# DavidBluecame/libYafaRay

Hardware: AMD Instinct MI355X
Metric: Mrays/sec + Msamples/sec, 1920×1080×64spp path-trace at 1/2/4/8 GPUs (higher is better)
Workload: dtype f32

## Files before the change

libyafaray_amd/csrc/devscene.h:

```cpp
#pragma once
#include <cstdint>
#include <hip/hip_runtime.h>

namespace yafamd
{
struct DevStats;

struct RadGrid
{
	const uint32_t *start;
	const float4 *pos;
	const float4 *dir;
	float lo[3];
	float cell, inv_cell;
	int nx, ny, nz;
};

enum : uint32_t
{
	B_NONE = 0, B_SPECULAR = 1u << 0, B_GLOSSY = 1u << 1, B_DIFFUSE = 1u << 2, B_DISPERSIVE = 1u << 3,
	B_REFLECT = 1u << 4, B_TRANSMIT = 1u << 5, B_FILTER = 1u << 6, B_EMIT = 1u << 7, B_VOLUMETRIC = 1u << 8,
	B_ALL = B_SPECULAR | B_GLOSSY | B_DIFFUSE | B_DISPERSIVE | B_REFLECT | B_TRANSMIT | B_FILTER
};

// ... 287 lines not shown
	float4 *pcol;
	float4 *pwo;
	float4 *pend_thr;
	float4 *pend_emit;
	float4 *v0p;
	float4 *v0wo;
	uint4 *pr;
	float4 *csmp;
	float *nee;
	float *nee_aw;
	uint8_t *occ;
	float4 *ts;
	float4 *v0attr;
};

struct DevQueues
{
	int *slot;
	float *ray_o;
	float *ray_d;
	float2 *ray_tt;
	float tmin_dflt;
	float *hit_t;
	int *hit_prim;
	float4 *sh_o;
	float4 *sh_d;
	int *sh_idx;
	float2 *ts_hit;
	int *ts_n;
	float4 *sattr;
	const uint32_t *perm;
	int trace_part;
	int nee_grid;
};

enum : int
{
	TRACE_BOTH = 0,
	TRACE_CLOSEST = 1,
	TRACE_SHADOW = 2,
};

struct DevNeeQueue
{
	float4 *p_prim;
	float4 *wo_k;
	uint4 *pix_mode;
	float4 *attr;
	float4 *extra;
};

enum : uint32_t
{
	G_DIFFUSE = 1u,
	G_CAUSTIC = 2u,
	G_EXTRA = 4u,
	G_FG = 8u,
	G_SHOWMAP = 16u,
};

struct PhotonState
{
	float4 *ray_o;
	float4 *ray_d;
	float4 *pcol;
	uint32_t *alive[2];
// ... 81 lines not shown
```

libyafaray_amd/csrc/kernels.hip:

```cpp

#include <atomic>
#include <hip/hip_runtime.h>
#include <cstdlib>
#include <string>
#include "devmath.h"
#include "photonheap.h"
#include "devscene.h"
#include "texeval.h"

namespace yafamd
{

#ifndef YAF_TRACE_BLOCK
#define YAF_TRACE_BLOCK 128
#endif
#ifndef YAF_SHADE_MIN_WAVES
#define YAF_SHADE_MIN_WAVES 4
#endif
#ifndef YAF_SHADE_LEAN_WAVES
#define YAF_SHADE_LEAN_WAVES 4
#endif
#ifndef YAF_SHADE_PREFETCH
#define YAF_SHADE_PREFETCH 1
#endif
// ... 761 lines not shown
			if(pk[1] != 0xffffffffu) { push((int)(pk[1] & nm)); ++sp; }
			next = pk[0] != 0xffffffffu ? (int)(pk[0] & nm) : -1;
		}
		else if constexpr(!YAF_CLOSEST_SORT)
		{
			int kmin = 0;
#pragma unroll
			for(int k = 1; k < 4; ++k) kmin = key[k] < key[kmin] ? k : kmin;
			next = key[kmin] < inf ? child[kmin] : -1;
#pragma unroll
			for(int k = 3; k >= 0; --k)
				if(k != kmin && key[k] < inf) { push(child[k]); ++sp; }
		}
		else
		{
			cswap(key[0], child[0], key[1], child[1]);
			cswap(key[2], child[2], key[3], child[3]);
			cswap(key[0], child[0], key[2], child[2]);
			cswap(key[1], child[1], key[3], child[3]);
			cswap(key[1], child[1], key[2], child[2]);
			if(key[3] < inf) { push(child[3]); ++sp; }
			if(key[2] < inf) { push(child[2]); ++sp; }
			if(key[1] < inf) { push(child[1]); ++sp; }
			next = key[0] < inf ? child[0] : -1;
		}
		if(next < 0)
		{
			if(sp == 0) break;
			--sp;
			next = (!SPILL || sp < C.lds_depth) ? C.stack[sp * kTraceBlock + YAF_LANE]
			                                    : C.spill[(uint32_t)(sp - C.lds_depth) * C.spill_stride + glane];
		}
		node = next;
	}
	return prim_best >= 0;
}

#undef YAF_LANE

template<bool SPILL, bool STATS = true>
__device__ void traceRefill4(const TraceCtx &C, const DevQueues &Q, const DevPaths &P, uint32_t n_a, uint32_t total,
                             uint32_t a0, uint32_t s0, uint32_t j, uint32_t stride, uint32_t &visits, uint32_t &tests,
                             uint32_t &n_closest, uint32_t &n_shadow)
{
	const int lane = threadIdx.x;
	const uint32_t glane = blockIdx.x * blockDim.x + threadIdx.x;
	const float inf = __builtin_huge_valf();
	V3 o = v3(0.f, 0.f, 0.f), d = o, id = o, oid = o;
	SlabSel sel{0, 2, 4};
	float tmin = 0.f, tmax = 0.f, box_t0 = 0.f, t_best = 0.f;
	int prim_best = -1, sp = 0, node = -1;
	bool any = false;
	uint32_t cur = 0;
	auto push = [&](int v) {
		if(sp < C.lds_depth) C.stack[sp * kTraceBlock + lane] = v;
		else if(SPILL) C.spill[(uint32_t)(sp - C.lds_depth) * C.spill_stride + glane] = v;
	};
	for(;;)
	{
		if(node < 0)
		{
			bool got = false;
			for(;;)
			{
				if(j >= total) break;
				cur = j;
// ... 396 lines not shown
	{
		const uint32_t k = key[r];
		uint64_t m = ~0ull;
#pragma unroll
		for(int b = 0; b < 6; ++b)
		{
			const bool bit = (k >> b) & 1u;
			const uint64_t bal = __ballot(bit);
			m &= bit ? bal : ~bal;
		}
		const uint32_t below = (uint32_t)__popcll(m & lt);
		const uint32_t old = W.base[k];
		off[r] = old + below;
		__builtin_amdgcn_wave_barrier();
		if(below == 0) W.base[k] = old + (uint32_t)__popcll(m);
		__builtin_amdgcn_wave_barrier();
	}
	const uint32_t c = W.base[lane];
	uint32_t inc = c;
#pragma unroll
	for(int o = 1; o < 64; o <<= 1)
	{
		const uint32_t v = __shfl_up(inc, o);
		if(lane >= o) inc += v;
	}
	__builtin_amdgcn_wave_barrier();
	W.base[lane] = inc - c;
	__builtin_amdgcn_wave_barrier();
#pragma unroll
	for(int r = 0; r < kSortPer; ++r) W.perm[W.base[key[r]] + off[r]] = (uint16_t)(r * 64 + lane);
	__builtin_amdgcn_wave_barrier();
}

template<bool LDS_SCENE, bool WIDE, bool TS, bool SPILL = true, bool STATS = true, bool SORT = false, bool W8 = false>
__global__ void __launch_bounds__(kTraceBlock) YAF_TRACE_ATTR k_trace(DevScene S, DevQueues Q, DevCounters cnt, DevPaths P,
                                                      DevStats *stats, int stack_depth, int *spill)
{
	extern __shared__ float4 smem[];
	int *stack = reinterpret_cast<int *>(smem);
	TraceCtx C;
	C.wave_base = waveBase();
	C.stack = stack;
	C.lds_depth = stack_depth;
	C.spill = spill;
	C.spill_stride = gridDim.x * blockDim.x;
	if(LDS_SCENE)
	{
		float4 *lds_nodes = smem + (stack_depth * kTraceBlock) / 4;
		float4 *lds_tris = lds_nodes + S.node_f4 * S.n_nodes;
		for(int k = threadIdx.x; k < S.node_f4 * S.n_nodes; k += blockDim.x) lds_nodes[k] = S.nodes[k];
		for(int k = threadIdx.x; k < 3 * S.n_tris; k += blockDim.x) lds_tris[k] = S.tris[k];
		__syncthreads();
		C.nodes = lds_nodes;
		C.tris = lds_tris;
	}
	else
	{
		C.nodes = S.nodes;
		C.tris = S.tris;
		if constexpr(W8)
		{
			C.nodes = S.nodes8;
			C.tris = S.tris8;
			if(S.lds_top8 > 0)
			{
				float4 *top = smem + (stack_depth * kTraceBlock) / 4;
				for(int k = threadIdx.x; k < 5 * S.lds_top8; k += blockDim.x) top[(k / 5) * kTop8Stride + (k % 5)] = S.nodes8[8 * (k / 5) + (k % 5)];
				__syncthreads();
				C.top = top;
				C.n_top = S.lds_top8;
			}
		}
		else if(WIDE && S.lds_top > 0)
		{
			float4 *top = smem + (stack_depth * kTraceBlock) / 4;
			for(int k = threadIdx.x; k < 8 * S.lds_top; k += blockDim.x) top[(k >> 3) * kTopStride + (k & 7)] = S.nodes[k];
			__syncthreads();
			C.top = top;
			C.n_top = S.lds_top;
		}
	}
	const SegLoop L = segLoop(S.n_seg);
	const uint32_t n_a = cnt.n_active[L.s], n_s = Q.trace_part == TRACE_CLOSEST ? 0u : cnt.n_shadow[L.s];
	const uint32_t total = n_a + n_s;
	const uint32_t j_first = Q.trace_part == TRACE_SHADOW ? n_a : 0u;
	const uint32_t a0 = L.s * S.cap_a, s0 = L.s * S.cap_s;
	uint32_t visits = 0, tests = 0, n_closest = 0, n_shadow = 0;
	uint32_t w_closest = 0, w_shadow = 0;
	auto countWave = [&](int kind) {
		w_closest += (uint32_t)__popcll(__ballot(kind == 1));
		w_shadow += (uint32_t)__popcll(__ballot(kind == 2));
	};
	const uint32_t stride = L.nb * blockDim.x;
	auto traceEntry = [&](uint32_t j) -> int {
		if(j < n_a)
		{
			const uint32_t i = a0 + j;
			V3 o, d;
			float tmin, tw;
			if(loadQRay(Q, i, o, d, tmin, tw))
			{
				float t;
				int prim;
				const float tmax = (tw >= 0.f) ? tw : __builtin_huge_valf();
				traverse<false, WIDE, SPILL, false, STATS, LDS_SCENE>(C, o, d, tmin, tmax, t, prim, visits, tests);
				raySt(&Q.hit_t[i], t);
				raySt(&Q.hit_prim[i], prim);
				return 1;
			}
		}
		else if(j < total)
		{
			const uint32_t k = s0 + (j - n_a);
			const float4 od = rayLd4(&Q.sh_o[k]), dd = rayLd4(&Q.sh_d[k]);
			float t;
			int prim;
			bool occ;
			if(TS)
			{
				TsList L;
				L.hit = Q.ts_hit + (size_t)k * (uint32_t)S.s_depth;
				L.n = 0;
				L.cap = S.s_depth;
				L.prim_ng = S.prim_ng;
				L.mats = S.mats;
				occ = traverse<true, WIDE, SPILL, true>(C, xyz(od), xyz(dd), od.w, dd.w, t, prim, visits, tests, &L);
				Q.ts_n[k] = occ ? 0 : L.n;
			}
			else occ = traverse<true, WIDE, SPILL, false, STATS>(C, xyz(od), xyz(dd), 0.f, dd.w, t, prim, visits, tests);
			P.occ[TS ? Q.sh_idx[k] : __float_as_int(od.w)] = occ ? 1 : 0;
			return 2;
		}
		return 0;
	};
	if constexpr(SORT)
	{
		__shared__ WaveSort wsort[kTraceBlock / 64];
		WaveSort &W = wsort[threadIdx.x >> 6];
		const uint32_t nwv = blockDim.x >> 6;
		const uint32_t gw = L.r * nwv + (threadIdx.x >> 6), nw = L.nb * nwv;
		for(uint32_t w0 = gw * kSortWin; w0 < total; w0 += nw * kSortWin)
		{
			uint32_t key[kSortPer];
#pragma unroll
			for(int r = 0; r < kSortPer; ++r)
			{
				const uint32_t j = w0 + (uint32_t)(r * 64) + laneId();
				uint32_t k = kSortBins - 1;
				if(j < n_a)
				{
					const F3 dd = reinterpret_cast<const F3 *>(Q.ray_d)[a0 + j];
					if(!(dd.x != dd.x)) k = rayKey(make_float4(dd.x, dd.y, dd.z, 0.f), false);
				}
				else if(j < total) k = rayKey(Q.sh_d[s0 + (j - n_a)], true);
				key[r] = k;
			}
			waveSortWindow(W, key);
#pragma unroll 1
			for(int r = 0; r < kSortPer; ++r) countWave(traceEntry(w0 + W.perm[r * 64 + laneId()]));
		}
	}
// ... 5019 lines not shown
	}
	return kStageErrWords;
}

int yafamd_experiments() { return kExperiments ? 1 : 0; }

#ifndef YAF_DEVICE_BUILD
#define YAF_DEVICE_BUILD "arch=? extra=[?] (built outside csrc/Makefile)"
#endif
const char *yafamd_device_build() { return YAF_DEVICE_BUILD
#ifdef YAF_PHASE_TIMING
	" phase-timing"
#endif
	; }

int yafamd_phase_cycles(unsigned long long *out, int n, int reset)
{
#ifdef YAF_PHASE_TIMING
	unsigned long long h[16];
	if(hipMemcpyFromSymbol(h, HIP_SYMBOL(g_phase), sizeof(h)) != hipSuccess) return 0;
	for(int k = 0; k < n && k < 16; ++k) out[k] = h[k];
	if(reset)
	{
		const unsigned long long z[16] = {};
		if(hipMemcpyToSymbol(HIP_SYMBOL(g_phase), z, sizeof(z)) != hipSuccess) return 0;
	}
	return 16;
#else
	(void)out; (void)n; (void)reset;
	return 0;
#endif
}

int yafamd_trace_blocks_per_cu(int lds_scene, int wide, size_t dyn_lds)
{
	int nb = 0;
	hipError_t e;
	if(wide == 8) e = hipOccupancyMaxActiveBlocksPerMultiprocessor(&nb, k_trace<false, true, false, true, false, false, true>, kTraceBlock, dyn_lds);
	else if(lds_scene) e = wide ? hipOccupancyMaxActiveBlocksPerMultiprocessor(&nb, k_trace<true, true, false>, kTraceBlock, dyn_lds)
	                       : hipOccupancyMaxActiveBlocksPerMultiprocessor(&nb, k_trace<true, false, false>, kTraceBlock, dyn_lds);
	else e = wide ? hipOccupancyMaxActiveBlocksPerMultiprocessor(&nb, k_trace<false, true, false>, kTraceBlock, dyn_lds)
	              : hipOccupancyMaxActiveBlocksPerMultiprocessor(&nb, k_trace<false, false, false>, kTraceBlock, dyn_lds);
	return e == hipSuccess ? nb : 0;
}

int yafamd_path_blocks_per_cu(const DevScene *S, int stack_depth)
{
	int nb = 0;
#ifdef YAF_EXPERIMENTS
	if(hipOccupancyMaxActiveBlocksPerMultiprocessor(&nb, k_path<false>, kTraceBlock, pathLdsBytes(*S, stack_depth)) != hipSuccess) nb = 0;
#else
	(void)S; (void)stack_depth;
#endif
	return nb;
}

int yafamd_nee_blocks_per_cu()
{
	int nb = 0;
	if(hipOccupancyMaxActiveBlocksPerMultiprocessor(&nb, (k_nee<true, false>), kShadeBlock, 8192) != hipSuccess) nb = 0;
	return nb;
}

int yafamd_shade_blocks_per_cu()
{
	int nb = 0;
	if(hipOccupancyMaxActiveBlocksPerMultiprocessor(&nb, (k_shade<true, false>), kShadeBlock, 8192) != hipSuccess) nb = 0;
	return nb;
}

hipError_t yafamd_launch_camera(const DevScene *S, const DevPaths *P, const DevQueues *Q, const DevCounters *cnt,
                                const DevJob *jobs, int n_jobs, uint64_t chunk_base, int n, int write_pr, hipStream_t st)
{
	if(n <= 0) return hipSuccess;
	const int threads = max(n, (int)S->n_seg);
	hipLaunchKernelGGL(k_camera, dim3((threads + 255) / 256), dim3(256), 0, st, *S, *P, *Q, *cnt, jobs, n_jobs, chunk_base, n, write_pr);
	return hipGetLastError();
}

hipError_t yafamd_launch_trace(const DevScene *S, const DevQueues *Q, const DevCounters *cnt, const DevPaths *P,
                               DevStats *stats, int stack_depth, int *spill, int grid, hipStream_t st)
{
	const size_t stack_bytes = (size_t)stack_depth * kTraceBlock * sizeof(int);
	const bool wide = S->node_f4 == 8;
	const size_t lds_scene = S->scene_in_lds ? (size_t)(S->node_f4 * S->n_nodes + 3 * S->n_tris) * sizeof(float4)
	                                         : (wide ? (size_t)S->lds_top * kTopStride * sizeof(float4) : 0);
	const size_t bytes = stack_bytes + lds_scene;
	if(S->nodes8 && !S->scene_in_lds && !S->tr_shad)
	{
		const size_t bytes8 = stack_bytes + (size_t)S->lds_top8 * kTop8Stride * sizeof(float4);
		if(S->trace_stats)
			hipLaunchKernelGGL((k_trace<false, true, false, true, true, false, true>), dim3(grid), dim3(kTraceBlock), bytes8, st, *S, *Q, *cnt, *P, stats,
			                   stack_depth, spill);
		else
			hipLaunchKernelGGL((k_trace<false, true, false, true, false, false, true>), dim3(grid), dim3(kTraceBlock), bytes8, st, *S, *Q, *cnt, *P, stats,
			                   stack_depth, spill);
		return hipGetLastError();
	}
#ifdef YAF_EXPERIMENTS
	if(S->brute && !S->tr_shad && S->n_tris <= kBruteTris)
	{
		hipLaunchKernelGGL(k_trace_brute, dim3(grid), dim3(kTraceBlock), 0, st, *S, *Q, *cnt, *P, stats);
		return hipGetLastError();
	}
#endif
#define YAF_TRACE_LAUNCH(L, W, T, SP) hipLaunchKernelGGL((k_trace<L, W, T, SP>), dim3(grid), dim3(kTraceBlock), bytes, st, *S, *Q, *cnt, *P, stats, stack_depth, spill)
	const bool nospill = spill == nullptr;
	if(S->tr_shad)
	{
		if(S->scene_in_lds)
		{
			if(nospill) { if(wide) YAF_TRACE_LAUNCH(true, true, true, false); else YAF_TRACE_LAUNCH(true, false, true, false); }
			else if(wide) YAF_TRACE_LAUNCH(true, true, true, true);
			else YAF_TRACE_LAUNCH(true, false, true, true);
		}
		else if(wide) YAF_TRACE_LAUNCH(false, true, true, true);
		else YAF_TRACE_LAUNCH(false, false, true, true);
	}
	else if(S->scene_in_lds)
	{
#ifdef YAF_EXPERIMENTS
		if(nospill && wide && S->ray_sort)
		{
			if(S->trace_stats)
				hipLaunchKernelGGL((k_trace<true, true, false, false, true, true>), dim3(grid), dim3(kTraceBlock), bytes, st, *S, *Q, *cnt, *P, stats,
				                   stack_depth, spill);
			else
				hipLaunchKernelGGL((k_trace<true, true, false, false, false, true>), dim3(grid), dim3(kTraceBlock), bytes, st, *S, *Q, *cnt, *P, stats,
				                   stack_depth, spill);
		}
		else
#endif
		if(nospill && wide && !S->trace_stats)
			hipLaunchKernelGGL((k_trace<true, true, false, false, false>), dim3(grid), dim3(kTraceBlock), bytes, st, *S, *Q, *cnt, *P, stats,
			                   stack_depth, spill);
		else if(nospill) { if(wide) YAF_TRACE_LAUNCH(true, true, false, false); else YAF_TRACE_LAUNCH(true, false, false, false); }
		else if(wide) YAF_TRACE_LAUNCH(true, true, false, true);
		else YAF_TRACE_LAUNCH(true, false, false, true);
	}
#ifdef YAF_EXPERIMENTS
	else if(wide && S->ray_sort)
	{
		if(S->trace_stats)
			hipLaunchKernelGGL((k_trace<false, true, false, true, true, true>), dim3(grid), dim3(kTraceBlock), bytes, st, *S, *Q, *cnt, *P, stats,
			                   stack_depth, spill);
		else
			hipLaunchKernelGGL((k_trace<false, true, false, true, false, true>), dim3(grid), dim3(kTraceBlock), bytes, st, *S, *Q, *cnt, *P, stats,
			                   stack_depth, spill);
	}
#endif
	else if(wide && !S->trace_stats)
		hipLaunchKernelGGL((k_trace<false, true, false, true, false>), dim3(grid), dim3(kTraceBlock), bytes, st, *S, *Q, *cnt, *P, stats,
		                   stack_depth, spill);
	else if(wide) YAF_TRACE_LAUNCH(false, true, false, true);
	else YAF_TRACE_LAUNCH(false, false, false, true);
#undef YAF_TRACE_LAUNCH
	return hipGetLastError();
}

hipError_t yafamd_launch_shade(const DevScene *S, const DevPaths *Pc, const DevPaths *Pn, const DevQueues *Q,
                               const DevQueues *Qn, const DevNeeQueue *N, const DevNeeQueue *G, const DevCounters *cnt,
                               const DevCounters *cnt_next, float4 *samples, const DevJob *jobs, int n_jobs, uint64_t chunk_base,
                               int stage_it, hipStream_t st)
{
	if(stage_it >= 0 && !(yafamd_shade_stages_for(S) && S->cur_level == 0 && S->lpc_mode == 0)) return hipErrorInvalidValue;
	ShadeArgs A;
// ... 603 lines not shown
```

libyafaray_amd/csrc/render.cc:

```cpp
#include "render.h"
#include "devmath.h"
#include "photonfile.h"

#include <hip/hip_runtime.h>
#include <rccl/rccl.h>

#include <algorithm>
#include <array>
#include <chrono>
#include <cmath>
#include <cstdlib>
#include <cstring>
#include <future>
#include <mutex>
#include <sstream>
#include <unordered_map>

using namespace yafamd;

extern "C" {
hipError_t yafamd_launch_camera(const DevScene *S, const DevPaths *P, const DevQueues *Q, const DevCounters *cnt,
                                const DevJob *jobs, int n_jobs, uint64_t chunk_base, int n, int write_pr, hipStream_t st);
hipError_t yafamd_launch_surface(const DevScene *S, const DevQueues *Q, const DevCounters *cnt, hipStream_t st);
hipError_t yafamd_launch_tshadow(const DevScene *S, const DevQueues *Q, const DevCounters *cnt, const DevPaths *P, hipStream_t st);
hipError_t yafamd_launch_spawn(const DevScene *S, const DevPaths *P, const DevQueues *Q, const DevCounters *cnt, uint32_t s0, int n,
                               hipStream_t st);
hipError_t yafamd_launch_combine(const DevScene *S, uint32_t lo, uint32_t hi, int final_level, float4 *samples, const DevJob *jobs,
                                 int n_jobs, uint64_t chunk_base, hipStream_t st);
hipError_t yafamd_launch_trace(const DevScene *S, const DevQueues *Q, const DevCounters *cnt, const DevPaths *P,
                               DevStats *stats, int stack_depth, int *spill, int grid, hipStream_t st);
int yafamd_trace_block();
int yafamd_shade_fused();
unsigned long long yafamd_xl_launches();
int yafamd_walk_lds_levels(int pm_stack);
int yafamd_walk_threads(const DevScene *S);
int yafamd_shade_fused_for(const DevScene *S);
int yafamd_experiments();
int yafamd_trace_blocks_per_cu(int lds_scene, int wide, size_t dyn_lds);
int yafamd_shade_blocks_per_cu();
hipError_t yafamd_launch_shade(const DevScene *S, const DevPaths *Pc, const DevPaths *Pn, const DevQueues *Q,
                               const DevQueues *Qn, const DevNeeQueue *N, const DevNeeQueue *G, const DevCounters *cnt,
                               const DevCounters *cnt_next, float4 *samples, const DevJob *jobs, int n_jobs, uint64_t chunk_base,
                               int stage_it, hipStream_t st);
int yafamd_shade_stages_for(const DevScene *S);
int yafamd_shade_stage_errors(uint32_t *out, int n);
int yafamd_path_eligible(const DevScene *S, int stack_depth, int spill);
int yafamd_path_blocks_per_cu(const DevScene *S, int stack_depth);
hipError_t yafamd_launch_path(const DevScene *S, float4 *samples, const DevJob *jobs, int n_jobs, uint64_t chunk_base, uint32_t n,
                              uint32_t *next, int stack_depth, int grid, hipStream_t st);
hipError_t yafamd_launch_nee(const DevScene *S, const DevNeeQueue *N, const DevPaths *Pn, const DevQueues *Qn,
                             const DevCounters *cnt_next, int stack_depth, hipStream_t st);
int yafamd_nee_blocks_per_cu();
hipError_t yafamd_photon_emit(const DevScene *S, const PhotonState *P, const PhotonSet *L, uint32_t n_photons, uint32_t h0, uint32_t n_local,
                              int max_bounces, hipStream_t st);
hipError_t yafamd_photon_bounce(const DevScene *S, const PhotonState *P, const PhotonSet *L, uint32_t n_photons, uint32_t h0,
                                uint32_t n_local, int max_bounces, int bounce, int cur, int stack_depth, int *spill, int grid, hipStream_t st);
hipError_t yafamd_photon_compact(const PhotonState *P, uint32_t *scratch_counts, uint32_t *total_dev, float4 *pos, float4 *dir, float *colb,
                                 hipStream_t st);
hipError_t yafamd_launch_gather(const DevScene *S, const DevNeeQueue *G, const DevCounters *cnt_next, float4 *samples,
                                const DevJob *jobs, int n_jobs, uint64_t chunk_base, const GatherLogDesc *log, hipStream_t st);
hipError_t yafamd_launch_gather_walk(const DevScene *S, const DevNeeQueue *G, const DevCounters *cnt_next, const GatherLogDesc *log,
                                     hipStream_t st);
int yafamd_gather_walk_k();
size_t yafamd_gather_lds_bytes(const DevScene *S);
hipError_t yafamd_rad_compact(const PhotonState *P, uint32_t *scratch_counts, uint32_t *total_dev, float4 *a, float4 *b, float4 *c, hipStream_t st);
hipError_t yafamd_rad_refl(const DevScene *S, float4 *a, float4 *b, float4 *c, const uint32_t *kept, uint32_t n, hipStream_t st);
hipError_t yafamd_pregather(const DevScene *S, const float4 *a, const float4 *b, const float4 *c, const uint32_t *kept, uint32_t n,
                            float4 *out_pos, float4 *out_dir, float *out_colb, DevStats *stats, hipStream_t st);
int yafamd_fg_paths_eligible(const DevScene *S);
hipError_t yafamd_launch_fg_paths(const DevScene *S, const DevNeeQueue *G, const DevCounters *cnt_next, int stack_depth, int *spill, int grid,
                                  const FgBatch *B, hipStream_t st);
// ... 20 lines not shown
                                  const float4 *src_attr, int n_out_verts, int n_out_prims, float *out_verts, int *out_tris, float4 *out_ng,
                                  float4 *out_attr, float *bounds, hipStream_t st);
hipError_t yafamd_build_pkd(const float4 *pos_dev, uint32_t n, uint4 *nodes_dev, int *depth_out, hipStream_t st, void **scratch);
hipError_t yafamd_build_pkd_kd(const float4 *pos_dev, const float4 *dir_dev, const float *colb_dev, uint32_t n, uint4 *nodes_dev, float4 *kpos,
                               float4 *kdir, float *kcolb, int *depth_out, hipStream_t st, void **scratch);
void yafamd_pkd_scratch_free(void *scratch);
hipError_t yafamd_build_pkd_kd_member(const float4 *pos_dev, const float4 *dir_dev, const float *colb_dev, uint32_t n, uint4 *nodes_dev, float4 *kpos,
                                      float4 *kdir, float *kcolb, int *depth_out, hipStream_t st, void **scratch, int member, int members,
                                      int *split_level);
void yafamd_pkd_top_segments(uint32_t n, int level, uint32_t *out);
void yafamd_pkd_owned_segments(int level, int member, int members, uint32_t *s0, uint32_t *s1);
hipError_t yafamd_pkd_parent_planes(uint4 *nodes_dev, uint32_t n, hipStream_t st);
hipError_t yafamd_launch_done_flags(const DevScene *S, const DevJob *jobs, int n_jobs, uint32_t n_pix, uint32_t done_pix, uint8_t *flags,
                                    hipStream_t st);
hipError_t yafamd_lpc_seg(const uint32_t *lpc, int W, int spp, int ts, int y0, int y1, uint32_t *seg, hipStream_t st);
hipError_t yafamd_lpc_prefix(uint32_t *lpc, int W, int spp, int ts, int y0, int y1, const uint32_t *segbase, hipStream_t st);
hipError_t yafamd_launch_film(const DevFilm *F, const float4 *samples, const uint8_t *flags, float4 *accum, float4 *out,
                              float *weights, int y0, int y1, float clamp_samples, int accumulate, hipStream_t st);
hipError_t yafamd_aa_next_pass(const float4 *accum, const float *weights, int W, int H, int tile, const DevAaParams *prm,
                               float threshold, uint8_t *flags, uint32_t *plist, uint32_t *count, int ry0, int ry1, uint32_t *local_count,
                               hipStream_t st);
hipError_t yafamd_launch_trace_rays(const DevScene *S, int any, const float4 *ro, const float4 *rd, int n, float *t_out,
                                    int *prim_out, int stack_depth, hipStream_t st);
hipError_t yafamd_layer_depth_range(const DevScene *S, float *range, int stack_depth, hipStream_t st);
hipError_t yafamd_launch_layer_hits(const DevScene *S, const DevLayers *L, const DevJob *jobs, int n_jobs, uint64_t chunk_base, int n, int stack_depth,
                                    hipStream_t st);
hipError_t yafamd_launch_layer_film(const DevFilm *F, const DevLayers *L, const float4 *prim_ng, const uint8_t *flags, float4 *accum, float4 *out,
                                    const float *weights, int y0, int y1, float clamp_samples, int accumulate, hipStream_t st);
}

namespace
{

struct DeviceGuard
{
	int prev = -1;
	bool set = false;
	explicit DeviceGuard(int dev)
	{
		if(dev >= 0 && hipGetDevice(&prev) == hipSuccess && prev != dev) set = hipSetDevice(dev) == hipSuccess;
	}
	~DeviceGuard()
	{
		if(set) (void)hipSetDevice(prev);
	}
};

struct Buf
{
	void *p = nullptr;
	size_t bytes = 0;
	void release()
	{
		if(p) (void)hipFree(p);
		p = nullptr;
		bytes = 0;
	}
};

std::vector<int> faurePerm(int b)
{
	if(b <= 2) return {0, 1};
	if((b & 1) == 0)
	{
		const std::vector<int> h = faurePerm(b / 2);
		std::vector<int> out;
// ... 132 lines not shown
	float light_inv_integral = 0.f;
	int n_ph_lights = 0;
	Buf cph_lights, clight_cdf, clight_func;
	float clight_inv_integral = 0.f;
	int n_cph_lights = 0;
	Buf cph_pos, cph_dir, cph_colb, cpk_nodes;
	Buf tile_rank, pfilm;
	Buf mesh_tris, mesh_cdf;
	Buf spot_pdf;
	Buf mesh_nodes, mesh_btris;
	int c_photons = 0, c_paths = 0, c_depth = 0;
	Buf ph_ray_o, ph_ray_d, ph_pcol, ph_alive0, ph_alive1, ph_n_alive, dep_a, dep_b, dep_c, dep_flag, ph_scan, ph_total;
	Buf ph_pos, ph_dir, ph_colb, pk_nodes, pk_stack;
	Buf rad_a, rad_b, rad_c, rad_flag, radc_a, radc_b, radc_c, rad_kept, rph_pos, rph_dir, rph_colb, rpk_nodes;
	Buf seg_pos, seg_dir, seg_colb, seg_ra, seg_rb, seg_rc;
	Buf fg_ts;
	Buf g_log, g_log_n;
	Buf walk_spill;
	Buf kd_pos[3], kd_dir[3], kd_colb[3];
	bool kd_on[3] = {false, false, false};
	int n_rphotons = 0;
	uint32_t n_rad_points = 0;
	int d_depth = 0, r_depth = 0;
	uint64_t map_owner[3] = {0, 0, 0};
	ncclComm_t comm = nullptr;
	Buf g_send, g_recv, g_wsend, g_wrecv, g_times, g_status;
	void *pkd_scratch = nullptr, *thin_scratch = nullptr, *rgrid_scratch = nullptr;
	std::vector<DevLight> host_lights;
	std::vector<DevLight> pass_lights;
	int n_photons = 0, pm_paths = 0, pm_stack = 0;
	uint32_t pm_local = 0;
	int n_nodes = 0, n_tris = 0, n_mats = 0, n_lights = 0, depth = 0, stack_depth = 32, node_f4 = 4;
	int lds_stack = 32;
	Buf spill;
	bool scene_in_lds = false;
	int lds_top = 0;
	int faure_bytes = 0;
	Buf samples, film, weights, jobs;
	Buf accum, aa_flags, aa_plist;
	int film_w = 0, film_h = 0;
	Buf lay_rec, lay_albedo, lay_accum, lay_film, lay_pfilm, lay_mat, lay_obj, lay_depth;
	int n_layers = 0;
	size_t slots_cap = 0;
	bool v0_alloc = false, tree_alloc = false, ao_alloc = false;
	int nee_cap = 0;
	std::vector<Buf> chunk_bufs;
	DevPaths P[2]{};
	DevQueues Q[2]{};
	Buf counters, stats;
	Buf path_next;
	Buf lpc, lpc_seg, lpc_stats;
	std::vector<hipEvent_t> ev_pool;
	bool prof_on = false;
	size_t ev_n = 2;
	struct ProfRec { int kind, e0, e1; };
	std::vector<ProfRec> prof_recs;
	hipEvent_t event(size_t i)
	{
		while(ev_pool.size() <= i)
		{
			hipEvent_t e = nullptr;
			if(hipEventCreate(&e) != hipSuccess) return nullptr;
			ev_pool.push_back(e);
		}
		return ev_pool[i];
	}
// ... 423 lines not shown
	if(const char *e = getenv("YAFARAY_AMD_LDS_STACK"); e && *e) d.lds_stack = std::min(d.stack_depth, std::max(4, atoi(e)));
	const size_t scene_bytes = (size_t)(d.node_f4 * d.n_nodes + 3 * d.n_tris) * 16;
	d.scene_in_lds = scene_bytes + (size_t)d.lds_stack * yafamd_trace_block() * 4 <= 48 * 1024;
	if(d.node_f4 == 8 && d.n_nodes >= 512) d.scene_in_lds = false;
	if(const char *e = getenv("YAFARAY_AMD_SCENE_LDS"); e && *e == '0') d.scene_in_lds = false;
	d.lds_top = 0;
	if(d.node_f4 == 8 && !d.scene_in_lds)
	{
		int top = 21;
		if(const char *e = getenv("YAFARAY_AMD_LDS_TOP"); e && *e) top = std::max(0, atoi(e));
		d.lds_top = std::min(top, d.n_nodes);
		const size_t stack_b = (size_t)d.lds_stack * yafamd_trace_block() * 4, lds_max = 64 * 1024;
		const int fit = stack_b >= lds_max ? 0 : (int)((lds_max - stack_b) / 144);
		if(d.lds_top > fit)
		{
			log_.warning("GPU: YAFARAY_AMD_LDS_TOP=" + std::to_string(d.lds_top) + " does not fit the trace workgroup's LDS; using " +
			             std::to_string(fit) + " nodes");
			d.lds_top = fit;
		}
	}
	d.lds_top8 = 0;
	if(d.nodes8.p && !d.scene_in_lds)
	{
		int top = 9;
		if(const char *e = getenv("YAFARAY_AMD_LDS_TOP8"); e && *e) top = std::max(0, atoi(e));
		const size_t stack_b = (size_t)d.lds_stack * yafamd_trace_block() * 4, lds_max = 64 * 1024;
		const int fit = stack_b >= lds_max ? 0 : (int)((lds_max - stack_b) / 80);
		d.lds_top8 = std::min(std::min(top, d.n_nodes8), fit);
	}
	{
		const bool w8 = d.nodes8.p && !d.scene_in_lds;
		const size_t dyn = (size_t)d.lds_stack * yafamd_trace_block() * 4 +
		                   (d.scene_in_lds ? scene_bytes : w8 ? (size_t)d.lds_top8 * 80 : (size_t)d.lds_top * 144);
		d.trace_grid = d.n_cu * std::max(1, yafamd_trace_blocks_per_cu(d.scene_in_lds ? 1 : 0, w8 ? 8 : (d.node_f4 == 8 ? 1 : 0), dyn));
		if(const char *e = getenv("YAFARAY_AMD_TRACE_GRID")) d.trace_grid = std::max(1, atoi(e));
		d.trace_grid = std::max(1, d.trace_grid / d.shade_grid) * d.shade_grid;
		d.trace_grid_bvh4 = d.trace_grid;
		if(w8 && !getenv("YAFARAY_AMD_TRACE_GRID"))
		{
			const size_t dyn4 = (size_t)d.lds_stack * yafamd_trace_block() * 4 + (size_t)d.lds_top * 144;
			int g4 = d.n_cu * std::max(1, yafamd_trace_blocks_per_cu(0, d.node_f4 == 8 ? 1 : 0, dyn4));
			g4 = std::max(1, g4 / d.shade_grid) * d.shade_grid;
			d.trace_grid_bvh4 = std::min(g4, d.trace_grid);
		}
	}
	d.spill.release();
	if(d.lds_stack < d.stack_depth &&
	   !ensure(log_, d.spill, (size_t)(d.stack_depth - d.lds_stack) * d.trace_grid * yafamd_trace_block() * sizeof(int)))
		return false;
	std::vector<uint8_t> perm;
	std::vector<uint32_t> off(50), base(50);
	std::vector<double> inv(50);
	int primes[50];
	primes[0] = 1;
	for(int k = 1, c = 2; k < 50; ++c)
	{
		bool pr = true;
		for(int q = 2; q * q <= c; ++q) if(c % q == 0) { pr = false; break; }
		if(pr) primes[k++] = c;
	}
	for(int dim = 0; dim < 50; ++dim)
	{
		const std::vector<int> p = faurePerm(dim <= 2 ? 3 : primes[dim]);
		off[dim] = (uint32_t)perm.size();
		for(int v : p) perm.push_back((uint8_t)v);
		base[dim] = (uint32_t)primes[dim];
		inv[dim] = (double)std::llround(1e9 / primes[dim]) / 1e9;
	}
	while(perm.size() % 16) perm.push_back(0);
	d.faure_bytes = (int)perm.size();
	if(!allocCopy(log_, d.faure, perm.data(), perm.size())) return false;
	std::vector<uint4> fdim(50);
	for(int dim = 0; dim < 50; ++dim)
	{
// ... 1253 lines not shown
	if(!ensure(log_, d.counters, 2 * 4 * R * sizeof(uint32_t))) return false;
	if(!ensure(log_, d.stats, sizeof(DevStats) * 2 * (size_t)d.trace_grid)) return false;
	HIPCHECK(hipMemsetAsync(d.counters.p, 0, 2 * 4 * R * sizeof(uint32_t), d.stream));
	HIPCHECK(hipMemsetAsync(d.stats.p, 0, sizeof(DevStats) * 2 * (size_t)d.trace_grid, d.stream));
	DevCounters cnt[2];
	for(int q = 0; q < 2; ++q)
	{
		uint32_t *base_q = (uint32_t *)d.counters.p + (size_t)q * 4 * R;
		cnt[q].n_active = base_q;
		cnt[q].n_shadow = base_q + R;
		cnt[q].n_nee = base_q + 2 * R;
		cnt[q].n_gather = base_q + 3 * R;
	}
	DevStats *dstats = (DevStats *)d.stats.p;
	S.stats = dstats;
	int nee_trace_stack = 0;
	{
		const char *ne = std::getenv("YAFARAY_AMD_NEE_TRACE");
		if(yafamd_experiments() && ne && std::string(ne) == "1" && d.lds_stack >= d.stack_depth) nee_trace_stack = d.lds_stack;
	}
	bool overlap = rp.device_sharers <= 1;
	int ov_nee_grid = std::max(1, (int)S.n_seg / 2), ov_trace_grid = std::max((int)S.n_seg, std::min(2 * (int)S.n_seg, d.trace_grid));
	if(const char *e = std::getenv("YAFARAY_AMD_OVERLAP"); e && *e) overlap = *e != '0';
	if(const char *e = std::getenv("YAFARAY_AMD_OVERLAP_NEE_GRID"); e && atoi(e) > 0) ov_nee_grid = atoi(e);
	if(const char *e = std::getenv("YAFARAY_AMD_OVERLAP_TRACE_GRID"); e && atoi(e) > 0)
		ov_trace_grid = (int)S.n_seg * std::max(1, std::min(atoi(e), d.trace_grid) / (int)S.n_seg);
	overlap = overlap && S.scene_in_lds && !S.ray_sort && !S.brute && !ray_bin && !S.tree && !S.tr_shad && !S.has_attr && nee_trace_stack == 0;
	bool ov_shadow = true;
	int ov_shadow_grid = d.trace_grid;
	if(const char *e = std::getenv("YAFARAY_AMD_OVERLAP_SHADOW"); e && *e) ov_shadow = *e != '0';
	if(const char *e = std::getenv("YAFARAY_AMD_OVERLAP_SHADOW_GRID"); e && atoi(e) > 0)
		ov_shadow_grid = (int)S.n_seg * std::max(1, std::min(atoi(e), d.trace_grid) / (int)S.n_seg);
	ov_shadow = ov_shadow && overlap && d.spill.p == nullptr;
	bool lpc_on = S.integrator == INT_PATH && S.n_lights > 1 && !S.tree && (rp.shard_world <= 1 || group_render);
	if(const char *lp = std::getenv("YAFARAY_AMD_LIGHT_PICK"); lp && std::string(lp) == "hash") lpc_on = false;
	lpc_carry_ = 0;
	S.lpc = nullptr;
	S.lpc_mode = 0;
	S.nee_pm16 = 0;
	if(const char *e = std::getenv("YAFARAY_AMD_NEE_PM16"); e && *e == '1') S.nee_pm16 = 1;
	if(const char *e = std::getenv("YAFARAY_AMD_W_LIVE"); e && *e == '1') S.w_live = 1;
	S.no_lean = 0;
	S.fg_probe = 0;
	if(const char *e = std::getenv("YAFARAY_AMD_FG_PROBE"); e && *e) S.fg_probe = atoi(e);
	if(const char *e = std::getenv("YAFARAY_AMD_SHADE_LEAN"); e && *e == '0') S.no_lean = 1;
	bool shade_stages = !lpc_on && yafamd_shade_stages_for(&S) != 0;
	if(const char *e = std::getenv("YAFARAY_AMD_SHADE_STAGES"); e && *e == '0') shade_stages = false;
	int path_grid = 0;
	if(!lpc_on)
	{
		const char *pe = std::getenv("YAFARAY_AMD_PATH");
		const bool on = yafamd_experiments() && pe && std::string(pe) == "mega";
		if(on && yafamd_path_eligible(&S, d.lds_stack, d.lds_stack < d.stack_depth ? 1 : 0))
		{
			path_grid = std::min(d.trace_grid, d.n_cu * std::max(1, yafamd_path_blocks_per_cu(&S, d.lds_stack)));
			if(const char *e = getenv("YAFARAY_AMD_PATH_GRID")) path_grid = std::min(d.trace_grid, std::max(1, atoi(e)));
			if(!ensure(log_, d.path_next, 16)) return false;
		}
	}
	const int n_paths = std::max(1, S.path_samples);
	const int iters = (S.integrator == INT_PATH) ? 2 + n_paths * (S.bounces + 2) : 3;

	auto ensureEvents = [&](size_t need) -> bool {
		while(d.ev_pool.size() < need)
		{
			hipEvent_t e;
			HIPCHECK(hipEventCreate(&e));
			d.ev_pool.push_back(e);
		}
		return true;
	};
	if(!ensureEvents(2)) return false;
	HIPCHECK(hipEventRecord(d.ev_pool[0], d.stream));
	DevStats *run_stats = dstats;
	bool shade_staged = false;
	auto iterate =[&](uint64_t base) -> bool {
		int cur = 0;
		const bool count_run = S.lpc_mode == 1;
		bool closest_done = false;
		for(int it = 0; it < iters; ++it)
		{
			DevQueues qc = d.Q[cur];
			if(it != 0 || (S.cur_level == 0 && !S.cam.ray_tt)) qc.ray_tt = nullptr;
			qc.tmin_dflt = it == 0 ? 0.f : S.ray_min_dist;
			qc.perm = nullptr;
			qc.trace_part = closest_done ? TRACE_SHADOW : TRACE_BOTH;
			const bool join_pending = closest_done && ov_shadow;
			closest_done = false;
			if(ray_bin && it >= 1 && !count_run)
			{
				size_t tb = d.bin_tmp.bytes;
				HIPCHECK(yafamd_ray_bin(&qc, &cnt[cur], S.n_seg, S.cap_a, d.scene_lo, d.scene_hi, (uint32_t *)d.bin_keys.p, (uint32_t *)d.bin_keys2.p,
				                        (uint32_t *)d.bin_iota.p, (uint32_t *)d.bin_perm.p, d.bin_tmp.p, &tb, d.stream));
				qc.perm = (const uint32_t *)d.bin_perm.p;
			}
			if(join_pending)
			{
				bool ok = [&]() -> bool {
					PROF(KK_TRACE, yafamd_launch_trace(&S, &qc, &cnt[cur], &d.P[cur], run_stats + d.trace_grid, d.lds_stack, nullptr, ov_shadow_grid,
					                                    d.stream));
					HIPCHECK(hipStreamWaitEvent(d.stream, d.ev_join, 0));
					return true;
				}();
				if(!ok)
				{
					(void)hipStreamSynchronize(d.side);
					return false;
				}
			}
			else
				PROF(KK_TRACE, yafamd_launch_trace(&S, &qc, &cnt[cur], &d.P[cur], run_stats, d.lds_stack, (int *)d.spill.p,
				                                    S.tr_shad ? d.trace_grid_bvh4 : d.trace_grid, d.stream));
			if(S.tr_shad && !count_run) PROF(KK_TSHADOW, yafamd_launch_tshadow(&S, &qc, &cnt[cur], &d.P[cur], d.stream));
			if(S.has_attr) PROF(KK_SURFACE, yafamd_launch_surface(&S, &qc, &cnt[cur], d.stream));
			if(S.lpc_mode == 3)
				HIPCHECK(yafamd_dfr_segoff(&cnt[cur], S.n_seg, (uint32_t *)d.dfr_segoff.p, (uint32_t *)d.dfr_misc.p, S.dfr_cap,
				                           (uint32_t *)d.dfr_misc.p + 1, (uint32_t *)d.dfr_its.p, d.stream));
			const int stage_it = (shade_stages && S.cur_level == 0 && S.lpc_mode == 0 && !S.tree) ? it : -1;
			PROF(KK_SHADE, yafamd_launch_shade(&S, &d.P[cur], &d.P[cur ^ 1], &qc, &d.Q[cur ^ 1], &d.N, &d.G, &cnt[cur], &cnt[cur ^ 1],
// ... 804 lines not shown
			}
	}
	constexpr uint8_t kOccUntouched = 0xEE;
	std::vector<uint8_t> occ((size_t)std::max(n_shadow, 1), kOccUntouched);

	Buf b_ro, b_rd, b_tt, b_ht, b_hp, b_so, b_sd, b_occ, b_na, b_ns, b_stats;
	bool ok = allocCopy(log_, b_ro, ro.data(), ro.size()) && allocCopy(log_, b_rd, rd.data(), rd.size()) &&
	          allocCopy(log_, b_tt, tt.data(), tt.size()) && allocCopy(log_, b_ht, ht.data(), ht.size()) &&
	          allocCopy(log_, b_hp, hp.data(), hp.size()) && allocCopy(log_, b_so, so.data(), so.size()) &&
	          allocCopy(log_, b_sd, sd.data(), sd.size()) && allocCopy(log_, b_occ, occ.data(), occ.size()) &&
	          allocCopy(log_, b_na, na.data(), na.size()) && allocCopy(log_, b_ns, ns.data(), ns.size()) &&
	          ensure(log_, b_stats, sizeof(DevStats) * (size_t)grid);
	std::vector<DevStats> per_block((size_t)grid);
	if(ok)
	{
		DevScene S{};
		fillScenePointers(d, S);
		S.n_seg = (uint32_t)n_seg;
		S.cap_a = cap_a;
		S.cap_s = cap_s;
		S.trace_stats = trace_stats ? 1 : 0;
		S.tr_shad = 0;
		DevQueues Q{};
		Q.ray_o = (float *)b_ro.p;
		Q.ray_d = (float *)b_rd.p;
		Q.ray_tt = need_tt ? (float2 *)b_tt.p : nullptr;
		Q.tmin_dflt = n_closest ? closest[6] : 0.f;
		Q.hit_t = (float *)b_ht.p;
		Q.hit_prim = (int *)b_hp.p;
		Q.sh_o = (float4 *)b_so.p;
		Q.sh_d = (float4 *)b_sd.p;
		Q.perm = nullptr;
		Q.trace_part = part;
		DevCounters cnt{};
		cnt.n_active = (uint32_t *)b_na.p;
		cnt.n_shadow = (uint32_t *)b_ns.p;
		DevPaths P{};
		P.occ = (uint8_t *)b_occ.p;
		ok = hipMemsetAsync(b_stats.p, 0, sizeof(DevStats) * (size_t)grid, d.stream) == hipSuccess &&
		     yafamd_launch_trace(&S, &Q, &cnt, &P, (DevStats *)b_stats.p, d.lds_stack, (int *)d.spill.p, grid, d.stream) == hipSuccess &&
		     hipStreamSynchronize(d.stream) == hipSuccess;
		if(!ok) log_.error("GPU: traceQueued: launch failed");
		ok = ok && hipMemcpy(ht.data(), b_ht.p, NA * sizeof(float), hipMemcpyDeviceToHost) == hipSuccess &&
		     hipMemcpy(hp.data(), b_hp.p, NA * sizeof(int), hipMemcpyDeviceToHost) == hipSuccess &&
		     hipMemcpy(occ.data(), b_occ.p, occ.size(), hipMemcpyDeviceToHost) == hipSuccess &&
		     hipMemcpy(per_block.data(), b_stats.p, sizeof(DevStats) * (size_t)grid, hipMemcpyDeviceToHost) == hipSuccess;
	}
	for(Buf *b : {&b_ro, &b_rd, &b_tt, &b_ht, &b_hp, &b_so, &b_sd, &b_occ, &b_na, &b_ns, &b_stats}) b->release();
	if(!ok) return false;
	for(int i = 0; i < n_closest; ++i) { t[i] = ht[qa[i]]; prim[i] = hp[qa[i]]; }
	for(int i = 0; i < n_shadow; ++i) if(occ[i] != kOccUntouched) occluded[i] = occ[i];
	if(counted)
	{
		counted[0] = counted[1] = 0;
		for(const DevStats &b : per_block) { counted[0] += b.closest_rays; counted[1] += b.shadow_rays; }
	}
	return true;
}


bool GpuRenderer::joinGroup(int rank, int world, const void *rccl_id, size_t id_bytes)
{
	if(!ready()) return false;
	DeviceGuard guard(device_);
	Impl &d = *d_;
	if(d.comm)
// ... 293 lines not shown
```

Baseline: 2302.

## Defer BVH4 leaf triangle tests into per-lane LDS list for LDS-resident scenes

Adds a BVH4 traversal variant that does not test leaf triangles when it reaches them. It records each leaf's start and count as a packed 16-bit entry in a per-lane LDS list and tests them in batches once the list fills or traversal ends. The aim is to cut wave divergence between node-box and triangle-test work, so lanes run the same phase together. In exchange it uses extra LDS sized to keep current occupancy, culls with a stale t_best during deferred phases, and only applies to small LDS-resident scenes with fewer than 1024 triangles. It is on by default for iterations after the first.

```diff
diff --git a/libyafaray_amd/csrc/devscene.h b/libyafaray_amd/csrc/devscene.h
--- a/libyafaray_amd/csrc/devscene.h
+++ b/libyafaray_amd/csrc/devscene.h
@@ -343,6 +343,7 @@
 	const uint32_t *perm;
 	int trace_part;
 	int nee_grid;
+	int trace_defer;
 };
 
 enum : int
diff --git a/libyafaray_amd/csrc/kernels.hip b/libyafaray_amd/csrc/kernels.hip
--- a/libyafaray_amd/csrc/kernels.hip
+++ b/libyafaray_amd/csrc/kernels.hip
@@ -817,6 +817,124 @@
 			                                    : C.spill[(uint32_t)(sp - C.lds_depth) * C.spill_stride + glane];
 		}
 		node = next;
+	}
+	return prim_best >= 0;
+}
+
+constexpr int kDeferStartBits = 10;
+constexpr int kDeferMaxLeaf = (1 << (16 - kDeferStartBits)) - 1;
+constexpr int kDeferRoom = 4;
+template<bool ANY, bool STATS>
+__device__ bool traverse4Defer(const TraceCtx &C, uint16_t *list, int cap, V3 o, V3 d, float tmin, float tmax, float &t_best,
+                               int &prim_best, uint32_t &visits, uint32_t &tests)
+{
+#if !YAF_LANE_REMAT
+	const int lane = threadIdx.x;
+#endif
+	V3 dd = d;
+	if(fabsf(dd.x) < 1e-20f) dd.x = copysignf(1e-20f, dd.x);
+	if(fabsf(dd.y) < 1e-20f) dd.y = copysignf(1e-20f, dd.y);
+	if(fabsf(dd.z) < 1e-20f) dd.z = copysignf(1e-20f, dd.z);
+	const V3 id = v3(rcpExact(dd.x), rcpExact(dd.y), rcpExact(dd.z));
+	const V3 oid = v3(o.x * id.x, o.y * id.y, o.z * id.z);
+	const SlabSel sel = slabSel(id);
+	const float box_t0 = ANY ? -1e-3f : (tmin - 1e-3f * (1.f + fabsf(tmin)));
+	const float inf = __builtin_huge_valf();
+	t_best = tmax;
+	prim_best = -1;
+	int sp = 0;
+	int node = 0;
+	int n = 0;
+	auto push = [&](int v) { C.stack[sp * kTraceBlock + YAF_LANE] = v; };
+	auto slackOf = [](float t) { return (t < 3.0e38f) ? t * 1.0000005f + 1e-6f : 3.4e38f; };
+	float slack_t = slackOf(t_best);
+	for(;;)
+	{
+		while(node >= 0 && n + kDeferRoom <= cap)
+		{
+			if(STATS) TRACE_STAT(++visits);
+			const float4 *np = C.nodes + 8 * node;
+			const float4 nx = np[sel.nx], fx = np[sel.nx ^ 1], ny = np[sel.ny], fy = np[sel.ny ^ 1], nz = np[sel.nz], fz = np[sel.nz ^ 1], cf = np[6], kf = np[7];
+			float key[4];
+			int child[4];
+			uint16_t *lp = list + n * kTraceBlock + YAF_LANE;
+#pragma unroll
+			for(int k = 0; k < 4; ++k)
+			{
+				const float lo = fmaxf(fmaxf(__builtin_fmaf(lane4(nx, k), id.x, -oid.x), __builtin_fmaf(lane4(ny, k), id.y, -oid.y)),
+				                       fmaxf(__builtin_fmaf(lane4(nz, k), id.z, -oid.z), box_t0));
+				const float hi = fminf(fminf(__builtin_fmaf(lane4(fx, k), id.x, -oid.x), __builtin_fmaf(lane4(fy, k), id.y, -oid.y)),
+				                       fminf(__builtin_fmaf(lane4(fz, k), id.z, -oid.z), slack_t));
+				const uint32_t h = lo <= hi ? 1u : 0u;
+				child[k] = __float_as_int(lane4(cf, k));
+				const int count = __float_as_int(lane4(kf, k));
+				const uint32_t inner = child[k] >= 0 ? 1u : 0u;
+				key[k] = (h & inner) ? lo : inf;
+				const uint32_t leaf = h & (inner ^ 1u) & (count > 0 ? 1u : 0u);
+				*lp = (uint16_t)((uint32_t)~child[k] | ((uint32_t)count << kDeferStartBits));
+				lp += leaf ? kTraceBlock : 0;
+				n += (int)leaf;
+			}
+			int next;
+			if constexpr(ANY && !YAF_ANY_SORT)
+			{
+				next = -1;
+#pragma unroll
+				for(int k = 0; k < 4; ++k)
+				{
+					if(!(key[k] < inf)) continue;
+					if(next < 0) next = child[k];
+					else { push(child[k]); ++sp; }
+				}
+			}
+			else
+			{
+				cswap(key[0], child[0], key[1], child[1]);
+				cswap(key[2], child[2], key[3], child[3]);
+				cswap(key[0], child[0], key[2], child[2]);
+				cswap(key[1], child[1], key[3], child[3]);
+				cswap(key[1], child[1], key[2], child[2]);
+				if(key[3] < inf) { push(child[3]); ++sp; }
+				if(key[2] < inf) { push(child[2]); ++sp; }
+				if(key[1] < inf) { push(child[1]); ++sp; }
+				next = key[0] < inf ? child[0] : -1;
+			}
+			if(next < 0 && sp > 0)
+			{
+				--sp;
+				next = C.stack[sp * kTraceBlock + YAF_LANE];
+			}
+			node = next;
+		}
+		uint32_t ent = 0;
+		for(;;)
+		{
+			if((ent >> kDeferStartBits) == 0)
+			{
+				if(n == 0) break;
+				--n;
+				ent = list[n * kTraceBlock + YAF_LANE];
+			}
+			if(STATS) TRACE_STAT(++tests);
+			const float4 *tp = C.tris + 3 * (ent & ((1u << kDeferStartBits) - 1u));
+			const float4 ta = tp[0], tb = tp[1], tc = tp[2];
+			ent += 1u - (1u << kDeferStartBits);
+			const float t = triTest(ta, tb, tc, o, d, ANY ? tmax : t_best);
+			if(t == -1.f) continue;
+			const int prim = __float_as_int(tb.w);
+			if(ANY)
+			{
+				if(t < tmax && t >= 0.f) { t_best = t; prim_best = prim; node = -1; break; }
+			}
+			else if(t >= tmin && (t < t_best || (t == t_best && prim_best >= 0 && prim < prim_best)))
+			{
+				t_best = t;
+				prim_best = prim;
+				slack_t = slackOf(t_best);
+			}
+		}
+		n = 0;
+		if(node < 0) break;
 	}
 	return prim_best >= 0;
 }
@@ -1279,10 +1397,11 @@
 	__builtin_amdgcn_wave_barrier();
 }
 
-template<bool LDS_SCENE, bool WIDE, bool TS, bool SPILL = true, bool STATS = true, bool SORT = false, bool W8 = false>
+template<bool LDS_SCENE, bool WIDE, bool TS, bool SPILL = true, bool STATS = true, bool SORT = false, bool W8 = false, bool DEFER = false>
 __global__ void __launch_bounds__(kTraceBlock) YAF_TRACE_ATTR k_trace(DevScene S, DevQueues Q, DevCounters cnt, DevPaths P,
                                                       DevStats *stats, int stack_depth, int *spill)
 {
+	static_assert(!DEFER || (LDS_SCENE && WIDE && !TS && !SPILL && !SORT && !W8), "deferred leaf tests: the plain no-spill BVH4 loop of LDS-resident scenes");
 	extern __shared__ float4 smem[];
 	int *stack = reinterpret_cast<int *>(smem);
 	TraceCtx C;
@@ -1291,6 +1410,7 @@
 	C.lds_depth = stack_depth;
 	C.spill = spill;
 	C.spill_stride = gridDim.x * blockDim.x;
+	uint16_t *dlist = nullptr;
 	if(LDS_SCENE)
 	{
 		float4 *lds_nodes = smem + (stack_depth * kTraceBlock) / 4;
@@ -1300,6 +1420,7 @@
 		__syncthreads();
 		C.nodes = lds_nodes;
 		C.tris = lds_tris;
+		if constexpr(DEFER) dlist = reinterpret_cast<uint16_t *>(lds_tris + 3 * S.n_tris);
 	}
 	else
 	{
@@ -1350,7 +1471,8 @@
 				float t;
 				int prim;
 				const float tmax = (tw >= 0.f) ? tw : __builtin_huge_valf();
-				traverse<false, WIDE, SPILL, false, STATS, LDS_SCENE>(C, o, d, tmin, tmax, t, prim, visits, tests);
+				if constexpr(DEFER) traverse4Defer<false, STATS>(C, dlist, Q.trace_defer, o, d, tmin, tmax, t, prim, visits, tests);
+				else traverse<false, WIDE, SPILL, false, STATS, LDS_SCENE>(C, o, d, tmin, tmax, t, prim, visits, tests);
 				raySt(&Q.hit_t[i], t);
 				raySt(&Q.hit_prim[i], prim);
 				return 1;
@@ -1374,6 +1496,7 @@
 				occ = traverse<true, WIDE, SPILL, true>(C, xyz(od), xyz(dd), od.w, dd.w, t, prim, visits, tests, &L);
 				Q.ts_n[k] = occ ? 0 : L.n;
 			}
+			else if constexpr(DEFER) occ = traverse4Defer<true, STATS>(C, dlist, Q.trace_defer, xyz(od), xyz(dd), 0.f, dd.w, t, prim, visits, tests);
 			else occ = traverse<true, WIDE, SPILL, false, STATS>(C, xyz(od), xyz(dd), 0.f, dd.w, t, prim, visits, tests);
 			P.occ[TS ? Q.sh_idx[k] : __float_as_int(od.w)] = occ ? 1 : 0;
 			return 2;
@@ -6459,11 +6582,15 @@
 #endif
 }
 
-int yafamd_trace_blocks_per_cu(int lds_scene, int wide, size_t dyn_lds)
+int yafamd_trace_defer_ok(int n_tris, int max_leaf) { return n_tris < (1 << kDeferStartBits) && max_leaf <= kDeferMaxLeaf; }
+int yafamd_trace_defer_min_cap() { return kDeferRoom; }
+
+int yafamd_trace_blocks_per_cu(int lds_scene, int wide, size_t dyn_lds, int defer)
 {
 	int nb = 0;
 	hipError_t e;
-	if(wide == 8) e = hipOccupancyMaxActiveBlocksPerMultiprocessor(&nb, k_trace<false, true, false, true, false, false, true>, kTraceBlock, dyn_lds);
+	if(defer) e = hipOccupancyMaxActiveBlocksPerMultiprocessor(&nb, k_trace<true, true, false, false, false, false, false, true>, kTraceBlock, dyn_lds);
+	else if(wide == 8) e = hipOccupancyMaxActiveBlocksPerMultiprocessor(&nb, k_trace<false, true, false, true, false, false, true>, kTraceBlock, dyn_lds);
 	else if(lds_scene) e = wide ? hipOccupancyMaxActiveBlocksPerMultiprocessor(&nb, k_trace<true, true, false>, kTraceBlock, dyn_lds)
 	                       : hipOccupancyMaxActiveBlocksPerMultiprocessor(&nb, k_trace<true, false, false>, kTraceBlock, dyn_lds);
 	else e = wide ? hipOccupancyMaxActiveBlocksPerMultiprocessor(&nb, k_trace<false, true, false>, kTraceBlock, dyn_lds)
@@ -6512,7 +6639,7 @@
 	const bool wide = S->node_f4 == 8;
 	const size_t lds_scene = S->scene_in_lds ? (size_t)(S->node_f4 * S->n_nodes + 3 * S->n_tris) * sizeof(float4)
 	                                         : (wide ? (size_t)S->lds_top * kTopStride * sizeof(float4) : 0);
-	const size_t bytes = stack_bytes + lds_scene;
+	size_t bytes = stack_bytes + lds_scene;
 	if(S->nodes8 && !S->scene_in_lds && !S->tr_shad)
 	{
 		const size_t bytes8 = stack_bytes + (size_t)S->lds_top8 * kTop8Stride * sizeof(float4);
@@ -6558,7 +6685,18 @@
 		}
 		else
 #endif
-		if(nospill && wide && !S->trace_stats)
+		if(nospill && wide && Q->trace_defer > 0)
+		{
+			if(Q->trace_defer < kDeferRoom || S->n_tris >= (1 << kDeferStartBits)) return hipErrorInvalidValue;
+			bytes += (size_t)Q->trace_defer * kTraceBlock * sizeof(uint16_t);
+			if(S->trace_stats)
+				hipLaunchKernelGGL((k_trace<true, true, false, false, true, false, false, true>), dim3(grid), dim3(kTraceBlock), bytes, st, *S, *Q, *cnt, *P, stats,
+				                   stack_depth, spill);
+			else
+				hipLaunchKernelGGL((k_trace<true, true, false, false, false, false, false, true>), dim3(grid), dim3(kTraceBlock), bytes, st, *S, *Q, *cnt, *P, stats,
+				                   stack_depth, spill);
+		}
+		else if(nospill && wide && !S->trace_stats)
 			hipLaunchKernelGGL((k_trace<true, true, false, false, false>), dim3(grid), dim3(kTraceBlock), bytes, st, *S, *Q, *cnt, *P, stats,
 			                   stack_depth, spill);
 		else if(nospill) { if(wide) YAF_TRACE_LAUNCH(true, true, false, false); else YAF_TRACE_LAUNCH(true, false, false, false); }
diff --git a/libyafaray_amd/csrc/render.cc b/libyafaray_amd/csrc/render.cc
--- a/libyafaray_amd/csrc/render.cc
+++ b/libyafaray_amd/csrc/render.cc
@@ -36,7 +36,9 @@
 int yafamd_walk_threads(const DevScene *S);
 int yafamd_shade_fused_for(const DevScene *S);
 int yafamd_experiments();
-int yafamd_trace_blocks_per_cu(int lds_scene, int wide, size_t dyn_lds);
+int yafamd_trace_blocks_per_cu(int lds_scene, int wide, size_t dyn_lds, int defer);
+int yafamd_trace_defer_ok(int n_tris, int max_leaf);
+int yafamd_trace_defer_min_cap();
 int yafamd_shade_blocks_per_cu();
 hipError_t yafamd_launch_shade(const DevScene *S, const DevPaths *Pc, const DevPaths *Pn, const DevQueues *Q,
                                const DevQueues *Qn, const DevNeeQueue *N, const DevNeeQueue *G, const DevCounters *cnt,
@@ -123,6 +125,14 @@
 namespace
 {
 
+constexpr bool kTraceDeferDefault = true;
+int traceDeferCap(int cap)
+{
+	bool on = kTraceDeferDefault;
+	if(const char *e = std::getenv("YAFARAY_AMD_TRACE_DEFER"); e && *e) on = *e != '0';
+	return on ? cap : 0;
+}
+
 struct DeviceGuard
 {
 	int prev = -1;
@@ -321,6 +331,7 @@
 	uint32_t pm_local = 0;
 	int n_nodes = 0, n_tris = 0, n_mats = 0, n_lights = 0, depth = 0, stack_depth = 32, node_f4 = 4;
 	int lds_stack = 32;
+	int trace_defer = 0;
 	Buf spill;
 	bool scene_in_lds = false;
 	int lds_top = 0;
@@ -810,14 +821,28 @@
 		const bool w8 = d.nodes8.p && !d.scene_in_lds;
 		const size_t dyn = (size_t)d.lds_stack * yafamd_trace_block() * 4 +
 		                   (d.scene_in_lds ? scene_bytes : w8 ? (size_t)d.lds_top8 * 80 : (size_t)d.lds_top * 144);
-		d.trace_grid = d.n_cu * std::max(1, yafamd_trace_blocks_per_cu(d.scene_in_lds ? 1 : 0, w8 ? 8 : (d.node_f4 == 8 ? 1 : 0), dyn));
+		const int per_cu = std::max(1, yafamd_trace_blocks_per_cu(d.scene_in_lds ? 1 : 0, w8 ? 8 : (d.node_f4 == 8 ? 1 : 0), dyn, 0));
+		d.trace_grid = d.n_cu * per_cu;
+		d.trace_defer = 0;
+		{
+			if(d.scene_in_lds && d.node_f4 == 8 && d.lds_stack >= d.stack_depth && yafamd_trace_defer_ok(d.n_tris, hs.bvh.max_leaf))
+			{
+				const int min_cap = yafamd_trace_defer_min_cap();
+				int cap = 8;
+				if(const char *e = getenv("YAFARAY_AMD_TRACE_DEFER_CAP"); e && *e) cap = atoi(e);
+				cap = std::min(std::max(cap, min_cap), 64);
+				auto fits = [&](int c) { return yafamd_trace_blocks_per_cu(1, 1, dyn + (size_t)c * yafamd_trace_block() * 2, 1) >= per_cu; };
+				while(cap > min_cap && !fits(cap)) cap = std::max(min_cap, cap - 2);
+				if(fits(cap)) d.trace_defer = cap;
+			}
+		}
 		if(const char *e = getenv("YAFARAY_AMD_TRACE_GRID")) d.trace_grid = std::max(1, atoi(e));
 		d.trace_grid = std::max(1, d.trace_grid / d.shade_grid) * d.shade_grid;
 		d.trace_grid_bvh4 = d.trace_grid;
 		if(w8 && !getenv("YAFARAY_AMD_TRACE_GRID"))
 		{
 			const size_t dyn4 = (size_t)d.lds_stack * yafamd_trace_block() * 4 + (size_t)d.lds_top * 144;
-			int g4 = d.n_cu * std::max(1, yafamd_trace_blocks_per_cu(0, d.node_f4 == 8 ? 1 : 0, dyn4));
+			int g4 = d.n_cu * std::max(1, yafamd_trace_blocks_per_cu(0, d.node_f4 == 8 ? 1 : 0, dyn4, 0));
 			g4 = std::max(1, g4 / d.shade_grid) * d.shade_grid;
 			d.trace_grid_bvh4 = std::min(g4, d.trace_grid);
 		}
@@ -2137,6 +2162,9 @@
 	if(const char *e = std::getenv("YAFARAY_AMD_OVERLAP_SHADOW_GRID"); e && atoi(e) > 0)
 		ov_shadow_grid = (int)S.n_seg * std::max(1, std::min(atoi(e), d.trace_grid) / (int)S.n_seg);
 	ov_shadow = ov_shadow && overlap && d.spill.p == nullptr;
+	d.Q[0].trace_defer = d.Q[1].trace_defer = traceDeferCap(d.trace_defer);
+	bool defer_it0 = false;
+	if(const char *e = std::getenv("YAFARAY_AMD_TRACE_DEFER_IT0"); e && *e) defer_it0 = *e != '0';
 	bool lpc_on = S.integrator == INT_PATH && S.n_lights > 1 && !S.tree && (rp.shard_world <= 1 || group_render);
 	if(const char *lp = std::getenv("YAFARAY_AMD_LIGHT_PICK"); lp && std::string(lp) == "hash") lpc_on = false;
 	lpc_carry_ = 0;
@@ -2190,6 +2218,7 @@
 			qc.tmin_dflt = it == 0 ? 0.f : S.ray_min_dist;
 			qc.perm = nullptr;
 			qc.trace_part = closest_done ? TRACE_SHADOW : TRACE_BOTH;
+			if(it == 0 && !defer_it0) qc.trace_defer = 0;
 			const bool join_pending = closest_done && ov_shadow;
 			closest_done = false;
 			if(ray_bin && it >= 1 && !count_run)
@@ -3060,6 +3089,7 @@
 		Q.sh_d = (float4 *)b_sd.p;
 		Q.perm = nullptr;
 		Q.trace_part = part;
+		Q.trace_defer = traceDeferCap(d.trace_defer);
 		DevCounters cnt{};
 		cnt.n_active = (uint32_t *)b_na.p;
 		cnt.n_shadow = (uint32_t *)b_ns.p;
```

After: 2438, median of 6. 5.9% higher.
